# autonomousvision/unimatch

Measured on AMD Instinct MI355X. Metric: image_pairs_per_sec, higher is better.
Workload: dtype f16x2

## Files before the change

include/unimatch_hip.h:

```cpp
#ifndef UNIMATCH_HIP_H
#define UNIMATCH_HIP_H

#include <stddef.h>
#include <stdint.h>

#ifdef __cplusplus
extern "C" {
#endif

#define UM_VERSION 220

#define UM_MODE_EXACT 0
#define UM_MODE_FAST 1

#define UM_ERR_BAD_ARG (-1)
#define UM_ERR_BAD_GEOMETRY (-2)
#define UM_ERR_WORKSPACE (-3)
#define UM_ERR_UNSUPPORTED (-4)
#define UM_ERR_COLLECTIVE (-5)

int um_version(void);
const char* um_last_error_string(void);

#define UM_RANGE_PLANES 1u
// ... 82 lines not shown

int um_linear_bias_fwd(const float* a0, const void* a_planes, const void* w_planes, const float* bias, int m, int n, int k,
                       int wshift, float out_mul, float bias_mul, void* out_planes, float* out_f32, int mode, void* stream);

int um_ffn_fwd(const float* x, const float* y, const void* w1_planes, const void* w2_planes, int m, int hidden,
               int wshift, const float* gamma, const float* beta, float eps, float* out, int mode, void* stream);
size_t um_ffn_split_workspace_bytes(int m, int hidden);
int um_ffn_ws_fwd(const float* x, const float* y, const void* w1_planes, const void* w2_planes, int m, int hidden,
                  int wshift, const float* gamma, const float* beta, float eps, float* out, int mode, void* workspace,
                  size_t workspace_bytes, void* stream);

int um_kv4_fwd(const float* x, const void* wc_planes, int m, int wshift, void* out_planes, int mode, void* stream);
int um_ffn_kv_fwd(const float* x, const float* y, const void* w1_planes, const void* w2_planes, int m, int hidden, int wshift,
                  const float* gamma, const float* beta, float eps, float* out, const void* wc_planes, void* kv_planes, int mode,
                  void* workspace, size_t workspace_bytes, void* stream);

int um_conv2d_fwd(const void* a_planes, const void* w_planes, const float* bias, float* out, float* stats_out, int batch,
                  int hi, int wi, int cin, int cout, int kh, int kw, int stride, int pad_h, int pad_w, int relu, int wshift,
                  int mode, void* stream);
int um_conv2d_ex(const void* a_planes, int a_ld, int a_coff, long a_rows, const void* w_planes, const float* bias, float* out,
                 int out_ld, int out_coff, void* out_planes, int outp_ld, int outp_coff, long outp_rows, float* stats_out,
                 int batch, int hi, int wi, int cin, int cout, int kh, int kw, int stride, int pad_h, int pad_w, int act,
                 int wshift, int mode, void* stream);
int um_conv2d_gru_fwd(int gate, const void* a_planes, int a_ld, int a_coff, long a_rows, const void* w_planes, const float* bias,
                      float* hidden, const float* z, int z_ld, float* z_out, int z_out_ld, void* out_planes, int outp_ld,
                      int outp_coff, long outp_rows, int batch, int hi, int wi, int cin, int channels, int kh, int kw, int pad_h,
                      int pad_w, int wshift, int mode, void* stream);
int um_conv2d_gru_add_fwd(int gate, const void* a_planes, int a_ld, int a_coff, long a_rows, const void* w_planes, const float* bias,
                          const float* addend, int addend_ld, float* hidden, const float* z, int z_ld, float* z_out, int z_out_ld,
                          void* out_planes, int outp_ld, int outp_coff, long outp_rows, int batch, int hi, int wi, int cin,
// ... 229 lines not shown
```

unimatch_amd/_abi.py:

```python
import ctypes
import os

_HERE = os.path.dirname(os.path.abspath(__file__))
LIB_PATH = os.environ.get('UM_LIB') or os.path.join(_HERE, 'libunimatch_hip.so')

MODE_EXACT = 0
MODE_FAST = 1

CENSUS = {'wattn_tile': 0, 'wattn_ksplit': 1, 'ffn_tile': 2, 'ffn_hsplit': 3, 'gsv4': 4, 'gsv3': 5, 'k4_mfma': 6, 'k4_valu': 7,
          'k3_mfma': 8, 'k3_valu': 9, 'conv_patch': 10, 'conv_rows': 11, 'conv_generic': 12, 'wattn_w8': 13, 'conv_patch_norm': 14}

_c_int, _c_size_t, _c_void_p = ctypes.c_int, ctypes.c_size_t, ctypes.c_void_p

SIGNATURES = {
    'um_version': (_c_int, []),
    'um_last_error_string': (ctypes.c_char_p, []),
    'um_range_flags': (_c_int, [ctypes.POINTER(ctypes.c_uint), _c_int]),
    'um_timing_enable': (_c_int, [_c_int]),
    'um_timing_collect': (_c_int, [_c_int, ctypes.POINTER(ctypes.c_double), ctypes.POINTER(_c_int)]),
    'um_window_attn_workspace_bytes': (_c_size_t, [_c_int] * 4),
    'um_window_attn_fwd': (_c_int, [_c_void_p] * 4 + [_c_int] * 9 + [_c_void_p, _c_size_t, _c_void_p]),
    'um_window_attn_planes_fwd': (_c_int, [_c_void_p] * 4 + [_c_int] * 6 + [ctypes.c_long] * 2 + [_c_int] * 6 + [_c_void_p]),
    'um_window_attn_merge_fwd': (_c_int, [_c_void_p] * 7 + [ctypes.c_float, _c_int, _c_void_p] + [_c_int] * 6 + [ctypes.c_long] * 2 +
                                 [_c_int] * 6 + [_c_void_p]),
    'um_window_attn_qproj_merge_fwd': (_c_int, [_c_void_p] * 8 + [ctypes.c_float, _c_int, _c_void_p] + [_c_int] * 5 + [ctypes.c_long] +
                                       [_c_int] * 6 + [_c_void_p, _c_size_t, _c_void_p]),
    'um_window_attn_ksplit_workspace_bytes': (_c_size_t, [_c_int] * 5),
    'um_window_attn_plan': (_c_int, [_c_int] * 5 + [ctypes.POINTER(_c_int)] * 3),
    'um_planes_bytes': (_c_size_t, [ctypes.c_long, _c_int, _c_int]),
    'um_weight_planes': (_c_int, [_c_void_p] * 2 + [_c_int] * 4 + [_c_void_p]),
    'um_linear_fwd': (_c_int, [_c_void_p] * 4 + [_c_int] * 5 + [_c_void_p] * 4 + [ctypes.c_float, _c_int, _c_void_p]),
    'um_linear_bias_fwd': (_c_int, [_c_void_p] * 4 + [_c_int] * 4 + [ctypes.c_float] * 2 + [_c_void_p] * 2 + [_c_int, _c_void_p]),
    'um_ffn_fwd': (_c_int, [_c_void_p] * 4 + [_c_int] * 3 + [_c_void_p] * 2 + [ctypes.c_float, _c_void_p, _c_int, _c_void_p]),
    'um_ffn_ws_fwd': (_c_int, [_c_void_p] * 4 + [_c_int] * 3 + [_c_void_p] * 2 + [ctypes.c_float, _c_void_p, _c_int, _c_void_p, _c_size_t,
                                _c_void_p]),
    'um_ffn_split_workspace_bytes': (_c_size_t, [_c_int] * 2),
    'um_ffn_kv_fwd': (_c_int, [_c_void_p] * 4 + [_c_int] * 3 + [_c_void_p] * 2 + [ctypes.c_float, _c_void_p, _c_void_p, _c_void_p, _c_int, _c_void_p,
                                _c_size_t, _c_void_p]),
    'um_kv4_fwd': (_c_int, [_c_void_p, _c_void_p, _c_int, _c_int, _c_void_p, _c_int, _c_void_p]),
    'um_conv2d_fwd': (_c_int, [_c_void_p] * 5 + [_c_int] * 13 + [_c_void_p]),
    'um_conv2d_addend_fwd': (_c_int, [_c_void_p] * 4 + [_c_int, _c_int, _c_void_p] + [_c_int] * 12 + [_c_void_p]),
    'um_conv2d_ex': (_c_int, [_c_void_p, _c_int, _c_int, ctypes.c_long, _c_void_p, _c_void_p, _c_void_p, _c_int, _c_int, _c_void_p,
                              _c_int, _c_int, ctypes.c_long, _c_void_p] + [_c_int] * 13 + [_c_void_p]),
    'um_nhwc_gate': (_c_int, [_c_int, _c_void_p, _c_int, _c_void_p, _c_void_p, _c_void_p, _c_int, _c_int, ctypes.c_long, ctypes.c_long,
                              _c_int, _c_void_p]),
    'um_local_corr_with_flow_planes': (_c_int, [_c_void_p] * 4 + [_c_int, ctypes.c_long] + [_c_int] * 5 + [_c_void_p]),
    'um_conv2d_gru_fwd': (_c_int, [_c_int, _c_void_p, _c_int, _c_int, ctypes.c_long, _c_void_p, _c_void_p, _c_void_p, _c_void_p, _c_int,
                                   _c_void_p, _c_int, _c_void_p, _c_int, _c_int, ctypes.c_long] + [_c_int] * 11 + [_c_void_p]),
    'um_conv2d_gru_add_fwd': (_c_int, [_c_int, _c_void_p, _c_int, _c_int, ctypes.c_long, _c_void_p, _c_void_p, _c_void_p, _c_int, _c_void_p, _c_void_p,
                                        _c_int, _c_void_p, _c_int, _c_void_p, _c_int, _c_int, ctypes.c_long] + [_c_int] * 11 + [_c_void_p]),
    'um_conv2d_norm_supported': (_c_int, [_c_int] * 10),
    'um_conv2d_norm_fwd': (_c_int, [_c_void_p, _c_void_p, _c_int] + [_c_void_p] * 4 + [_c_int] * 13 + [_c_void_p]),
    'um_conv2d_entry_supported': (_c_int, [_c_int] * 10),
# ... 188 lines not shown
```

unimatch_amd/csrc/ffn.hip:

```cpp
#include <type_traits>
#include <stdlib.h>
#include "common.h"
#include "planes.h"

#ifdef UM_FFN_TRACE
__device__ unsigned long long* g_um_ffn_trace = nullptr;
#define UM_FSTAMP(slot) do { if (tracing && i < 24) trace_buf[(i) * 8 + (slot)] = __builtin_amdgcn_s_memtime(); } while (0)
#else
#define UM_FSTAMP(slot) do { } while (0)
#endif

struct Kv4Args {
    const float* x;
    const unsigned short* w;
    long w_plane_stride;
    unsigned short* out;
    long out_plane_stride;
    int M;
    float out_scale;
    unsigned* range_flag;
};

struct FfnArgs {
    const float* x;
// ... 1 lines not shown
    const unsigned short* w1;
    long w1_plane_stride;
    const unsigned short* w2;
    long w2_plane_stride;
    const float* gamma;
    const float* beta;
    float* out;
    int M, hid;
    float out_scale;
    float eps;
    int split;
    float* hs_part;
    unsigned* hs_flag;
    Kv4Args kv;
    unsigned* range_flag;
};

#ifndef UM_FFN_PRIO
#define UM_FFN_PRIO 0
#endif
#ifndef UM_FFN_ABL
#define UM_FFN_ABL 0
#endif
struct Gelu2 {
    float x[2], r[2];
};
#define UM_GELU_STAGES 4
__device__ __forceinline__ void ffn_gelu_stage(Gelu2& g, int stage) {
#pragma unroll
    for (int i = 0; i < 2; ++i) {
// ... 168 lines not shown
            if (NS == 2) {
                const u32x4 l = {T::lo2(v0[0], v0[1], h[0], neg1), T::lo2(v0[2], v0[3], h[1], neg1),
                                 T::lo2(v1[0], v1[1], h[2], neg1), T::lo2(v1[2], v1[3], h[3], neg1)};
                yf[NS - 1][ks] = __builtin_bit_cast(i16x8, l);
            }
        }
        um_range_note<T>(k.range_flag, xmx, UM_RANGE_KV_TOKENS);
    }
    const int arow = tl ^ (16 * role);
    int aoff[8];
#pragma unroll
    for (int ks = 0; ks < 8; ++ks) aoff[ks] = arow * 512 + (((16 * role + 2 * ks + half) ^ arow) << 4);
    kv4_project<T, NS, false>(lds, lds + Kv4Lds<NS>::RING, k, yf, m0, wave, lane, aoff, neg1);
}

template <typename T, int NS, bool HSPLIT = false, bool KV4 = false>
__global__ __launch_bounds__(512, 2) void ffn_kernel(FfnArgs a) {
    using L = FfnLds<NS>;
    extern __shared__ __attribute__((aligned(16))) unsigned char lds[];

    const int tid = threadIdx.x, lane = tid & 63;
    const float neg1 = um_opaque_neg1();
    const int wave = __builtin_amdgcn_readfirstlane(tid >> 6);
    const int pair = wave & 3, role = wave >> 2;
    const int half = lane >> 5, tl = lane & 31;
    const int nsplit = HSPLIT ? a.split : 1;
    const int tile_id = HSPLIT ? (int)blockIdx.x / nsplit : (int)blockIdx.x;
    const int part = HSPLIT ? (int)blockIdx.x - tile_id * nsplit : 0;
    const int m0 = tile_id * 128;
    const int tok = m0 + 32 * pair + tl;
    const int nslice = (a.hid >> 5) / nsplit;
// ... 489 lines not shown
            for (int g = 0; g < 4; ++g) {
                const int n = 32 * ot + 8 * g;
                const f32x4 gm = *reinterpret_cast<const f32x4*>(a.gamma + n + 4 * half);
                const f32x4 bt = *reinterpret_cast<const f32x4*>(a.beta + n + 4 * half);
                f32x4 yv;
#pragma unroll
                for (int i = 0; i < 4; ++i) yv[i] = (o[ot][4 * g + i] - mean) * rstd * gm[i] + bt[i] + rr[4 * ot + g][i];
                *reinterpret_cast<f32x4*>(stg + tl * 512 + (((8 * ot + 2 * g + half) ^ tl) << 4)) = yv;
                if constexpr (KV4) {
#pragma unroll
                    for (int i = 0; i < 4; ++i) o[ot][4 * g + i] = yv[i];
                }
            }
        __builtin_amdgcn_wave_barrier();
        const int cc = lane & 31;
#pragma unroll
        for (int j = 0; j < 16; ++j) {
            const int r = 2 * j + half;
            const f32x4 v = *reinterpret_cast<const f32x4*>(stg + r * 512 + ((cc ^ r) << 4));
            const int trow = m0 + 32 * pair + r;
            if (trow < a.M) *reinterpret_cast<f32x4*>(a.out + (long)trow * 128 + 4 * cc) = v;
        }
    }
#ifdef UM_FFN_TRACE
    if (tracing) trace_buf[24 * 8 + 2] = __builtin_amdgcn_s_memtime();
#endif
    if constexpr (KV4) {
        i16x8 yf[NS][8];
        unsigned char* xch = lds + 65536 + pair * 16384 + lane * 16;
        if (role == 0) {
#pragma unroll
            for (int ot = 0; ot < 4; ++ot)
#pragma unroll
                for (int kk = 0; kk < 2; ++kk) {
                    unsigned wh[4], wl[4];
#pragma unroll
                    for (int j = 0; j < 4; ++j) {
// ... 28 lines not shown
        }
        kv4_project<T, NS, true>(lds, lds + 65536, a.kv, yf, m0, wave, lane, aoff, neg1);
#ifdef UM_FFN_TRACE
        if (tracing) trace_buf[24 * 8 + 3] = __builtin_amdgcn_s_memtime();
#endif
    }
}

extern void um_set_error(const char* fmt, ...);
#ifdef UM_FFN_TRACE
extern "C" int um_debug_set_ffn_trace(void* ptr) {
    return (int)hipMemcpyToSymbol(HIP_SYMBOL(g_um_ffn_trace), &ptr, sizeof(ptr));
}
#endif

template <typename T, int NS, bool HSPLIT, bool KV4 = false>
static hipError_t launch_ffn_impl(const FfnArgs& a, hipStream_t stream) {
    constexpr int LDS = FfnLds<NS>::TOTAL > 131072 ? FfnLds<NS>::TOTAL : (KV4 ? 131072 : FfnLds<NS>::TOTAL);
    static bool configured = false;
    if (!configured) {
        hipError_t e = hipFuncSetAttribute(reinterpret_cast<const void*>(&ffn_kernel<T, NS, HSPLIT, KV4>),
                                           hipFuncAttributeMaxDynamicSharedMemorySize, LDS);
        if (e != hipSuccess) return e;
        configured = true;
    }
    ScopedKernelTimer timer(UM_K_FFN, stream);
    um_census_hit(HSPLIT ? UM_V_FFN_HSPLIT : UM_V_FFN_TILE);
    hipLaunchKernelGGL((ffn_kernel<T, NS, HSPLIT, KV4>), dim3(((a.M + 127) / 128) * a.split), dim3(512), LDS, stream, a);
    return hipGetLastError();
}

template <typename T, int NS>
static hipError_t launch_ffn(const FfnArgs& a, hipStream_t stream) {
    if (a.kv.w) return launch_ffn_impl<T, NS, false, true>(a, stream);
    return a.split > 1 ? launch_ffn_impl<T, NS, true>(a, stream) : launch_ffn_impl<T, NS, false>(a, stream);
}

static int ffn_num_cus() { return um_num_cus(); }

static int ffn_hidden_split(int m, int hidden) {
    static const bool off = um_debug_env("UM_FFN_NO_HSPLIT") != nullptr;
    if (off) return 1;
    const int tiles = (m + 127) / 128, nslice = hidden / 32, cus = ffn_num_cus();
    int split = 1;
    while (split < 4 && tiles * (2 * split) <= cus && nslice % (2 * split) == 0 && nslice / (2 * split) >= 4) split *= 2;
    return split;
}

static size_t ffn_hs_bytes(int m, int split) {
// ... 8 lines not shown
}

extern "C" int um_ffn_ws_fwd(const float* x, const float* y, const void* w1_planes, const void* w2_planes, int m, int hidden,
                             int wshift, const float* gamma, const float* beta, float eps, float* out, int mode, void* workspace,
                             size_t workspace_bytes, void* stream_);

extern "C" int um_ffn_fwd(const float* x, const float* y, const void* w1_planes, const void* w2_planes, int m, int hidden,
                          int wshift, const float* gamma, const float* beta, float eps, float* out, int mode,
                          void* stream_) {
    return um_ffn_ws_fwd(x, y, w1_planes, w2_planes, m, hidden, wshift, gamma, beta, eps, out, mode, nullptr, 0, stream_);
}

extern "C" int um_kv4_fwd(const float* x, const void* wc_planes, int m, int wshift, void* out_planes, int mode, void* stream_);
static int ffn_impl(const float* x, const float* y, const void* w1_planes, const void* w2_planes, int m, int hidden,
                    int wshift, const float* gamma, const float* beta, float eps, float* out, int mode, void* workspace,
                    size_t workspace_bytes, const void* wc_planes, void* kv_planes, void* stream_);

extern "C" int um_ffn_ws_fwd(const float* x, const float* y, const void* w1_planes, const void* w2_planes, int m, int hidden,
                             int wshift, const float* gamma, const float* beta, float eps, float* out, int mode, void* workspace,
                             size_t workspace_bytes, void* stream_) {
    return ffn_impl(x, y, w1_planes, w2_planes, m, hidden, wshift, gamma, beta, eps, out, mode, workspace, workspace_bytes, nullptr,
                    nullptr, stream_);
}

extern "C" int um_ffn_kv_fwd(const float* x, const float* y, const void* w1_planes, const void* w2_planes, int m, int hidden,
                             int wshift, const float* gamma, const float* beta, float eps, float* out, const void* wc_planes,
                             void* kv_planes, int mode, void* workspace, size_t workspace_bytes, void* stream_) {
    if (!wc_planes || !kv_planes) {
        um_set_error("um_ffn_kv_fwd: null k | v weight planes or output planes");
        return -1;
    }
    return ffn_impl(x, y, w1_planes, w2_planes, m, hidden, wshift, gamma, beta, eps, out, mode, workspace, workspace_bytes, wc_planes,
                    kv_planes, stream_);
}

static int ffn_impl(const float* x, const float* y, const void* w1_planes, const void* w2_planes, int m, int hidden,
                    int wshift, const float* gamma, const float* beta, float eps, float* out, int mode, void* workspace,
                    size_t workspace_bytes, const void* wc_planes, void* kv_planes, void* stream_) {
    if (!x || !y || !w1_planes || !w2_planes || !gamma || !beta || !out || m <= 0 || hidden < 64 || hidden % 32 != 0 ||
        (mode != 0 && mode != 1) || wshift < 0 || wshift > 14) {
        um_set_error("um_ffn_fwd: bad argument (m=%d hidden=%d wshift=%d mode=%d; hidden must be a multiple of 32, >= 64)",
                     m, hidden, wshift, mode);
        return -1;
    }
    if ((long)hidden * 256 * 2 >= (1L << 32)) {
        um_set_error("um_ffn_fwd: weight planes beyond 4 GiB are not addressable by this kernel");
        return -4;
    }
    FfnArgs a;
    a.x = x;
    a.y = y;
    a.w1 = (const unsigned short*)w1_planes;
    a.w1_plane_stride = (long)hidden * 256;
    a.w2 = (const unsigned short*)w2_planes;
    a.w2_plane_stride = (long)128 * hidden;
    a.gamma = gamma;
    a.beta = beta;
    a.out = out;
    a.M = m;
    a.hid = hidden;
    a.out_scale = ldexpf(1.f, -wshift);
    a.eps = eps;
    a.split = 1;
    a.hs_part = nullptr;
    a.hs_flag = nullptr;
    a.kv = Kv4Args{};
    a.range_flag = a.kv.range_flag = (mode == 0) ? um_range_flag_dev() : nullptr;
    if (workspace) {
        const int split = ffn_hidden_split(m, hidden);
        if (split > 1 && workspace_bytes >= ffn_hs_bytes(m, split)) {
            const size_t slots = (size_t)((m + 127) / 128);
            a.split = split;
            a.hs_flag = (unsigned*)workspace;
            a.hs_part = (float*)((unsigned char*)workspace + ((slots * sizeof(unsigned) + 255) & ~(size_t)255));
        }
    }
    static const bool no_fuse = um_debug_env("UM_FFN_NO_KV4") != nullptr;
    const bool fuse = wc_planes && a.split == 1 && !no_fuse;
    if (fuse) {
        a.kv.x = nullptr;
        a.kv.w = (const unsigned short*)wc_planes;
        a.kv.w_plane_stride = 256L * 256;
        a.kv.out = (unsigned short*)kv_planes;
        a.kv.out_plane_stride = 4L * m * 128;
        a.kv.M = m;
        a.kv.out_scale = a.out_scale;
    }
    const hipError_t e = mode == 0 ? launch_ffn<Fp16, 2>(a, (hipStream_t)stream_) : launch_ffn<Bf16, 1>(a, (hipStream_t)stream_);
    if (e != hipSuccess) {
        um_set_error("um_ffn_fwd: launch failed: %s", hipGetErrorString(e));
        return (int)e;
    }
    if (wc_planes && !fuse) return um_kv4_fwd(out, wc_planes, m, wshift, kv_planes, mode, stream_);
    return 0;
}

extern "C" int um_kv4_fwd(const float* x, const void* wc_planes, int m, int wshift, void* out_planes, int mode, void* stream_) {
    if (!x || !wc_planes || !out_planes || m <= 0 || (mode != 0 && mode != 1) || wshift < 0 || wshift > 14) {
        um_set_error("um_kv4_fwd: bad argument (m=%d wshift=%d mode=%d)", m, wshift, mode);
        return -1;
    }
    Kv4Args k;
    k.x = x;
    k.w = (const unsigned short*)wc_planes;
    k.w_plane_stride = 256L * 256;
    k.out = (unsigned short*)out_planes;
    k.out_plane_stride = 4L * m * 128;
    k.M = m;
// ... 32 lines not shown
```

unimatch_amd/model.py:

```python
import math
import weakref

import torch
import torch.nn as nn
import torch.nn.functional as F

from .encoder import CNNEncoder
from .refine import BasicUpdateBlock, convex_upsample
from .refine_nhwc import NhwcUpdateBlock
from .dist import shard_batch, shard_bounds
from .streams import PartRunner, forward_parts
from .confidence import depth_match_confidence, match_confidence

_IMAGENET_MEAN = (0.485, 0.456, 0.406)
_IMAGENET_STD = (0.229, 0.224, 0.225)


def attention_windows(attn_type, is_self, splits, h, w, with_shift):
    if attn_type == 'swin':
        kind = 'win2d'
    elif attn_type == 'self_swin2d_cross_1d':
        kind = 'win2d' if is_self else 'row'
    elif attn_type == 'self_swin2d_cross_swin1d':
        kind = 'win2d' if is_self else 'winrow'
# ... 40 lines not shown
class TransformerLayer(nn.Module):

    def __init__(self, d_model, no_ffn, ffn_dim_expansion):
        super().__init__()
        self.q_proj = nn.Linear(d_model, d_model, bias=False)
        self.k_proj = nn.Linear(d_model, d_model, bias=False)
        self.v_proj = nn.Linear(d_model, d_model, bias=False)
        self.merge = nn.Linear(d_model, d_model, bias=False)
        self.norm1 = nn.LayerNorm(d_model)
        self.no_ffn = no_ffn
        if not no_ffn:
            self.mlp = nn.Sequential(nn.Linear(2 * d_model, 2 * d_model * ffn_dim_expansion, bias=False), nn.GELU(),
                                     nn.Linear(2 * d_model * ffn_dim_expansion, d_model, bias=False))
            self.norm2 = nn.LayerNorm(d_model)

    def forward(self, ops, source, target, h, w, geom, kv_rotate=0, kv=None, next_kv_weights=None):
        if getattr(ops, 'fused_tail', False):
            return self._forward_fused(ops, source, target, h, w, geom, kv_rotate, kv, next_kv_weights)
        assert kv_rotate == 0 and kv is None and next_kv_weights is None
        q, k, v = self.q_proj(source), self.k_proj(target), self.v_proj(target)
        msg = ops.window_attention(q, k, v, h, w, *geom)
        msg = self.norm1(self.merge(msg))
        if not self.no_ffn:
            msg = self.norm2(self.mlp(torch.cat([source, msg], dim=-1)))
        return source + msg

    def _forward_fused(self, ops, source, target, h, w, geom, kv_rotate=0, kv=None, next_kv_weights=None):
        s, l, c = source.shape
        m = s * l
        src = source.reshape(m, c)
        if getattr(ops, 'fused_qproj', False) and getattr(ops, 'fused_merge', False):
            if kv is None:
                kvp, _, n2 = ops.linear_planes(target.reshape(m, c), (self.k_proj.weight, self.v_proj.weight))
                koff, voff = 0, c
                kop, vop = (kvp, m, n2, koff), (kvp, m, n2, voff)
            else:
                kop, vop = kv
                assert kop[1] == m
            res = src if self.no_ffn else None
            msg = ops.window_attention_qproj_merge(src, self.q_proj.weight, kop, vop, s, h, w, *geom,
                                                   kv_rotate, self.merge.weight, self.norm1, res)
            if self.no_ffn:
                return msg
            msg = msg.reshape(m, c)
            if next_kv_weights is not None:
                out, nkv = ops.ffn_ln_kv(src, msg, self.mlp[0].weight, self.mlp[2].weight, self.norm2, next_kv_weights)
                return out.reshape(s, l, c), nkv
            if getattr(ops, 'fused_ffn', False):
                return ops.ffn_ln(src, msg, self.mlp[0].weight, self.mlp[2].weight, self.norm2).reshape(s, l, c)
            hid, _, nh = ops.linear_planes(src, (self.mlp[0].weight,), a1=msg, gelu=True)
            return ops.linear_ln(hid, (self.mlp[2].weight,), self.norm2, residual=src, a_planes_k=nh).reshape(s, l, c)
        assert kv is None and next_kv_weights is None, 'precomputed k | v planes need the fused q-projection / merge path'
        if target is source:
            qkv, _, n3 = ops.linear_planes(src, (self.q_proj.weight, self.k_proj.weight, self.v_proj.weight))
            q, k, v = (qkv, m, n3, 0), (qkv, m, n3, c), (qkv, m, n3, 2 * c)
        else:
            qp, _, _ = ops.linear_planes(src, (self.q_proj.weight,))
            kv, _, n2 = ops.linear_planes(target.reshape(m, c), (self.k_proj.weight, self.v_proj.weight))
            q, k, v = (qp, m, c, 0), (kv, m, n2, 0), (kv, m, n2, c)
        if getattr(ops, 'fused_merge', False):
            res = src if self.no_ffn else None
            msg = ops.window_attention_merge(q, k, v, s, h, w, *geom, kv_rotate, self.merge.weight, self.norm1, res)
            if self.no_ffn:
                return msg
            msg = msg.reshape(m, c)
        else:
            att = ops.window_attention_planes(q, k, v, s, h, w, *geom, kv_rotate=kv_rotate).reshape(m, c)
# ... 20 lines not shown
        if nhead != 1:
            raise NotImplementedError('multi-head attention is not implemented (neither does the reference, '
                                      'transformer.py:63-66)')
        self.d_model = d_model
        self.layers = nn.ModuleList([TransformerBlock(d_model, ffn_dim_expansion) for _ in range(num_layers)])
        for p in self.parameters():
            if p.dim() > 1:
                nn.init.xavier_uniform_(p)

    def forward(self, ops, tok0, tok1, h, w, attn_type, attn_num_splits, stream=None):
        if stream is None:
            stream = torch.cat([tok0, tok1], 0)
        b = stream.shape[0] // 2
        rotate = getattr(ops, 'fused_tail', False)
        prev = stream if rotate else torch.cat([stream[b:], stream[:b]], 0)
        block_kv = rotate and getattr(ops, 'fused_qproj', False) and getattr(ops, 'fused_merge', False) and getattr(ops, 'block_kv', True)
        s2, l, c = stream.shape
        fused_kv = block_kv and getattr(ops, 'fused_kv', False) and getattr(ops, 'fused_ffn', False)
        kv4 = None
        kvw = lambda b_: (b_.self_attn.k_proj.weight, b_.self_attn.v_proj.weight, b_.cross_attn_ffn.k_proj.weight,
                          b_.cross_attn_ffn.v_proj.weight)
        for i, blk in enumerate(self.layers):
            shift = ('swin' in attn_type) and attn_num_splits > 1 and i % 2 == 1
            g_self = attention_windows(attn_type, True, attn_num_splits, h, w, shift)
            g_cross = attention_windows(attn_type, False, attn_num_splits, h, w, shift)
            kv_s = kv_c = None
            if block_kv:
                if kv4 is None:
                    kv4 = ops.kv4_planes(stream.reshape(s2 * l, c), kvw(blk))
                kv_s, kv_c = ops.kv4_slices(kv4, s2 * l)
                kv4 = None
            stream = blk.self_attn(ops, stream, stream, h, w, g_self, kv=kv_s)
            if rotate:
                nxt = kvw(self.layers[i + 1]) if fused_kv and i + 1 < len(self.layers) else None
                stream = blk.cross_attn_ffn(ops, stream, prev, h, w, g_cross, kv_rotate=b, kv=kv_c, next_kv_weights=nxt)
                if nxt is not None:
                    stream, kv4 = stream
                prev = stream
            else:
                stream = blk.cross_attn_ffn(ops, stream, prev, h, w, g_cross)
                prev = torch.cat([stream[b:], stream[:b]], 0)
        return stream[:b].contiguous(), stream[b:].contiguous()


class SelfAttnPropagation(nn.Module):

    def __init__(self, in_channels):
        super().__init__()
        self.q_proj = nn.Linear(in_channels, in_channels)
        self.k_proj = nn.Linear(in_channels, in_channels)
        for p in self.parameters():
            if p.dim() > 1:
# ... 811 lines not shown
```

unimatch_amd/ops.py:

```python
import contextlib
import ctypes
import threading
import weakref
from collections import namedtuple

import torch

from . import _abi

PRECISIONS = {'exact': _abi.MODE_EXACT, 'fast': _abi.MODE_FAST}


class KernelTimer:

    def __init__(self):
        self.records = []

    def summary(self):
        torch.cuda.synchronize()
        out = {}
        for name, s, e, meta in self.records:
            d = out.setdefault(name, {'calls': 0, 'ms': 0.0, 'meta': meta})
            d['calls'] += 1
            d['ms'] += s.elapsed_time(e)
# ... 16 lines not shown
        raise ValueError(f'{name}: shape {tuple(t.shape)} does not match N={n}, L={tokens}')


def _check_map(name, t, n, h, w):
    if not (t.is_cuda and t.dtype == torch.float32 and t.dim() == 4 and t.is_contiguous()
            and t.shape[0] == n and t.shape[2] == h and t.shape[3] == w):
        raise ValueError(f'{name}: expected a contiguous CUDA float32 [{n}, V, {h}, {w}] tensor, got '
                         f'{tuple(t.shape)} {t.dtype}')


def pack_kv4_weights(weights):
    w4 = torch.cat([w.detach().float() for w in weights], 0)
    perm = torch.arange(32, device=w4.device) ^ 16
    cross = w4[256:].view(8, 32, 128)[:, perm].reshape(256, 128)
    return torch.cat([w4[:256], cross], 1).contiguous()


WorkspaceKey = namedtuple('WorkspaceKey', 'kind geometry device owner')


class _Scope(threading.local):
    token = None
    lane = 0


class WorkspaceRegistry:

    GEOMETRIES = 8

    def __init__(self, stream=None, capturing=None):
# ... 41 lines not shown
        return buf

    def release_cached_planes(self):
        for k in [k for k in self._entries if isinstance(k.kind, tuple)]:
            del self._entries[k]


class HipOps(WorkspaceRegistry):

    fused_tail = True
    fused_ffn = True
    fused_merge = True
    fused_qproj = True
    block_kv = True
    refine_hoist = True
    fused_kv = True
    fused_conv = True
    norm_on_load = True
    fused_entry = True
    fused_glue = True
    CONV_MODE = 0
    WSHIFT = 10

    def __init__(self, precision='exact'):
        if precision not in PRECISIONS:
            raise ValueError(f'precision must be one of {sorted(PRECISIONS)}')
        self.lib = _abi.load()
        if not torch.cuda.is_available():
            raise _abi.HipExtensionError('no GPU visible: the UniMatch hot path only runs on the HIP extension')
        self.precision = precision
        self.mode = PRECISIONS[precision]
# ... 53 lines not shown
        self.cache_generation += 1
        return value

    def weight_planes(self, weights):
        key, hit = self._cache_get('lin', weights)
        if hit is not None:
            return hit
        w = (weights[0] if len(weights) == 1 else torch.cat(list(weights), 0)).detach().float().contiguous()
        n, k = w.shape
        self._check_weight_range(w, self.WSHIFT if self.mode == 0 else 0, 'Linear weight')
        planes = torch.empty(self.lib.um_planes_bytes(n, k, self.mode), dtype=torch.uint8, device=w.device)
        _abi.check(self.lib.um_weight_planes(_ptr(w), _ptr(planes), n, k, self.WSHIFT, self.mode, _stream()),
                   'um_weight_planes')
        return self._cache_put(key, weights, (planes, n, k))

    @staticmethod
    def _check_weight_range(w, shift, what):
        limit = 65504.0 / float(1 << shift)
        amax = float(w.abs().max()) if w.numel() else 0.0
        if not amax < limit:
            raise ValueError(f'{what}: max |w| = {amax:.4g} does not fit the fp16 operand planes (|w| < {limit:.4g} at the '
                             f'2^{shift} pre-scale; see include/unimatch_hip.h, "Operand range")')

    def _check_rows(self, name, t, k):
        if not (t.is_cuda and t.dtype == torch.float32 and t.dim() == 2 and t.is_contiguous() and t.shape[1] == k):
            raise ValueError(f'{name}: expected a contiguous CUDA float32 [M, {k}] tensor, got {tuple(t.shape)} {t.dtype}')

    def linear_planes(self, a, weights, a1=None, gelu=False, a_planes_k=None):
        wp, n, k = self.weight_planes(weights)
        if a_planes_k is not None:
            m = a.numel() // (2 * self.nplanes * a_planes_k)
            args = (None, None, _ptr(a))
        else:
            m = a.shape[0]
            self._check_rows('a', a, k // 2 if a1 is not None else k)
            if a1 is not None:
                self._check_rows('a1', a1, k // 2)
            args = (_ptr(a), _ptr(a1) if a1 is not None else None, None)
        out = torch.empty(self.lib.um_planes_bytes(m, n, self.mode), dtype=torch.uint8, device=a.device)
        meta = {'flops': 2.0 * m * n * k}
        code = self._launch('linear', lambda: self.lib.um_linear_fwd(
            args[0], args[1], args[2], _ptr(wp), m, n, k, self.WSHIFT, 2 if gelu else 0, _ptr(out),
            None, None, None, 0.0, self.mode, _stream()), meta)
# ... 7 lines not shown
            args = (None, None, _ptr(a))
        else:
            m = a.shape[0]
            self._check_rows('a', a, k)
            args = (_ptr(a), None, None)
        if residual is not None:
            self._check_rows('residual', residual, n)
        out = torch.empty((m, n), dtype=torch.float32, device=a.device)
        code = self._launch('linear', lambda: self.lib.um_linear_fwd(
            args[0], args[1], args[2], _ptr(wp), m, n, k, self.WSHIFT, 1, _ptr(out),
            _ptr(norm.weight), _ptr(norm.bias), _ptr(residual) if residual is not None else None,
            float(norm.eps), self.mode, _stream()), {'flops': 2.0 * m * n * k})
        _abi.check(code, 'um_linear_fwd')
        return out

    def ffn_ln(self, x, y, w1, w2, norm):
        w1p, hid, k1 = self.weight_planes((w1,))
        w2p, n2, k2 = self.weight_planes((w2,))
        if (k1, n2, k2) != (256, 128, hid):
            raise ValueError(f'ffn_ln: expected W1 [hidden, 256] and W2 [128, hidden], got {tuple(w1.shape)} {tuple(w2.shape)}')
        self._check_rows('x', x, 128)
        self._check_rows('y', y, 128)
        m = x.shape[0]
        if y.shape[0] != m:
            raise ValueError('ffn_ln: x and y must have the same number of rows')
        out = torch.empty((m, 128), dtype=torch.float32, device=x.device)
        ws = self._split_workspace('ffn_hsplit', (m, hid), x.device)
        code = self._launch('ffn', lambda: self.lib.um_ffn_ws_fwd(
            _ptr(x), _ptr(y), _ptr(w1p), _ptr(w2p), m, hid, self.WSHIFT, _ptr(norm.weight), _ptr(norm.bias),
            float(norm.eps), _ptr(out), self.mode, _ptr(ws) if ws is not None else None, ws.numel() if ws is not None else 0,
            _stream()), {'flops': 2.0 * m * hid * (256 + 128)})
        _abi.check(code, 'um_ffn_ws_fwd')
        return out

    def ffn_ln_kv(self, x, y, w1, w2, norm, kv_weights):
        w1p, hid, k1 = self.weight_planes((w1,))
        w2p, n2, k2 = self.weight_planes((w2,))
        if (k1, n2, k2) != (256, 128, hid):
            raise ValueError(f'ffn_ln_kv: expected W1 [hidden, 256] and W2 [128, hidden], got {tuple(w1.shape)} {tuple(w2.shape)}')
        self._check_rows('x', x, 128)
        self._check_rows('y', y, 128)
        m = x.shape[0]
# ... 36 lines not shown
        out = torch.empty((streams, h * w, 128), dtype=torch.float32, device=qt.device)
        meta = {'flops': 4.0 * streams * h * w * win_h * win_w * 128}
        code = self._launch('window_attn', lambda: self.lib.um_window_attn_merge_fwd(
            _ptr(qt) + 2 * qoff, _ptr(kt) + 2 * koff, _ptr(vt) + 2 * voff, _ptr(wp), _ptr(norm.weight), _ptr(norm.bias),
            _ptr(residual) if residual is not None else None, float(norm.eps), self.WSHIFT, _ptr(out), streams, h, w, 128,
            qcols, kcols, qrows * qcols, krows * kcols, win_h, win_w, shift_h, shift_w, kv_rotate, self.mode, _stream()), meta)
        _abi.check(code, 'um_window_attn_merge_fwd')
        return out

    def _split_workspace(self, kind, geometry, device):
        size = self.lib.um_window_attn_ksplit_workspace_bytes if kind == 'attn_ksplit' else self.lib.um_ffn_split_workspace_bytes
        nbytes = size(*geometry)
        return self._workspace(kind, geometry, nbytes, device, self.GEOMETRIES) if nbytes else None

    def window_attention_qproj_merge(self, x, q_weight, k, v, streams, h, w, win_h, win_w, shift_h, shift_w, kv_rotate,
                                     merge_weight, norm, residual=None):
        (kt, krows, kcols, koff), (vt, vrows, vcols, voff) = k[:4], v[:4]
        kps = k[4] if len(k) > 4 else krows * kcols
        if (v[4] if len(v) > 4 else vrows * vcols) != kps:
            raise ValueError('k and v must share their plane stride')
        self._check_rows('x', x, 128)
        if (krows, kcols) != (vrows, vcols) or x.shape[0] != streams * h * w or krows != x.shape[0]:
            raise ValueError('inconsistent plane shapes')
        wqp, nq, kq = self.weight_planes((q_weight,))
        wp, n, kk = self.weight_planes((merge_weight,))
        if (n, kk, nq, kq) != (128, 128, 128, 128):
            raise ValueError('window_attention_qproj_merge: the query and merge weights must be [128, 128]')
        if residual is not None:
            self._check_rows('residual', residual, 128)
        out = torch.empty((streams, h * w, 128), dtype=torch.float32, device=x.device)
        meta = {'flops': 4.0 * streams * h * w * win_h * win_w * 128}
        ks = self._split_workspace('attn_ksplit', (streams, h, w, win_h, win_w), x.device)
        code = self._launch('window_attn', lambda: self.lib.um_window_attn_qproj_merge_fwd(
            _ptr(x), _ptr(wqp), _ptr(kt) + 2 * koff, _ptr(vt) + 2 * voff, _ptr(wp), _ptr(norm.weight), _ptr(norm.bias),
            _ptr(residual) if residual is not None else None, float(norm.eps), self.WSHIFT, _ptr(out), streams, h, w, 128,
            kcols, kps, win_h, win_w, shift_h, shift_w, kv_rotate, self.mode,
            _ptr(ks) if ks is not None else None, ks.numel() if ks is not None else 0, _stream()), meta)
        _abi.check(code, 'um_window_attn_qproj_merge_fwd')
# ... 916 lines not shown
```

Baseline: 983.6.

## Fold K/V projections into query and merge weights, emit FFN output planes

Folds the key projection into the query weight (Wk^T·Wq) and the value projection into the merge weight (Wm·Wv), so attention reads the raw stream planes and no per-layer K/V projection GEMM is needed. The FFN kernel gains a PLANES variant that writes fp16/bf16 split planes of its output in the epilogue, and these become the next layer's K/V input. The folded layer path is turned on by default and the fused_kv path is turned off. The folded weights are computed in double precision and cached, but reassociating the products changes rounding and may raise the dynamic range that the plane quantisation must cover.

Result: faster. 1034, median of 6 (+5.2%).

```diff
diff --git a/include/unimatch_hip.h b/include/unimatch_hip.h
--- a/include/unimatch_hip.h
+++ b/include/unimatch_hip.h
@@ -120,6 +120,9 @@
 int um_ffn_kv_fwd(const float* x, const float* y, const void* w1_planes, const void* w2_planes, int m, int hidden, int wshift,
                   const float* gamma, const float* beta, float eps, float* out, const void* wc_planes, void* kv_planes, int mode,
                   void* workspace, size_t workspace_bytes, void* stream);
+int um_ffn_planes_fwd(const float* x, const float* y, const void* w1_planes, const void* w2_planes, int m, int hidden, int wshift,
+                      const float* gamma, const float* beta, float eps, float* out, void* out_planes, int mode, void* workspace,
+                      size_t workspace_bytes, void* stream);
 
 int um_conv2d_fwd(const void* a_planes, const void* w_planes, const float* bias, float* out, float* stats_out, int batch,
                   int hi, int wi, int cin, int cout, int kh, int kw, int stride, int pad_h, int pad_w, int relu, int wshift,
diff --git a/unimatch_amd/_abi.py b/unimatch_amd/_abi.py
--- a/unimatch_amd/_abi.py
+++ b/unimatch_amd/_abi.py
@@ -37,6 +37,8 @@
     'um_ffn_split_workspace_bytes': (_c_size_t, [_c_int] * 2),
     'um_ffn_kv_fwd': (_c_int, [_c_void_p] * 4 + [_c_int] * 3 + [_c_void_p] * 2 + [ctypes.c_float, _c_void_p, _c_void_p, _c_void_p, _c_int, _c_void_p,
                                 _c_size_t, _c_void_p]),
+    'um_ffn_planes_fwd': (_c_int, [_c_void_p] * 4 + [_c_int] * 3 + [_c_void_p] * 2 + [ctypes.c_float, _c_void_p, _c_void_p, _c_int, _c_void_p, _c_size_t,
+                                    _c_void_p]),
     'um_kv4_fwd': (_c_int, [_c_void_p, _c_void_p, _c_int, _c_int, _c_void_p, _c_int, _c_void_p]),
     'um_conv2d_fwd': (_c_int, [_c_void_p] * 5 + [_c_int] * 13 + [_c_void_p]),
     'um_conv2d_addend_fwd': (_c_int, [_c_void_p] * 4 + [_c_int, _c_int, _c_void_p] + [_c_int] * 12 + [_c_void_p]),
diff --git a/unimatch_amd/csrc/ffn.hip b/unimatch_amd/csrc/ffn.hip
--- a/unimatch_amd/csrc/ffn.hip
+++ b/unimatch_amd/csrc/ffn.hip
@@ -39,6 +39,8 @@
     unsigned* hs_flag;
     Kv4Args kv;
     unsigned* range_flag;
+    unsigned short* planes;
+    long planes_stride;
 };
 
 #ifndef UM_FFN_PRIO
@@ -237,7 +239,7 @@
     kv4_project<T, NS, false>(lds, lds + Kv4Lds<NS>::RING, k, yf, m0, wave, lane, aoff, neg1);
 }
 
-template <typename T, int NS, bool HSPLIT = false, bool KV4 = false>
+template <typename T, int NS, bool HSPLIT = false, bool KV4 = false, bool PLANES = false>
 __global__ __launch_bounds__(512, 2) void ffn_kernel(FfnArgs a) {
     using L = FfnLds<NS>;
     extern __shared__ __attribute__((aligned(16))) unsigned char lds[];
@@ -757,13 +759,25 @@
             }
         __builtin_amdgcn_wave_barrier();
         const int cc = lane & 31;
+        float pmx = 0.f;
 #pragma unroll
         for (int j = 0; j < 16; ++j) {
             const int r = 2 * j + half;
             const f32x4 v = *reinterpret_cast<const f32x4*>(stg + r * 512 + ((cc ^ r) << 4));
             const int trow = m0 + 32 * pair + r;
-            if (trow < a.M) *reinterpret_cast<f32x4*>(a.out + (long)trow * 128 + 4 * cc) = v;
-        }
+            if (trow < a.M) {
+                *reinterpret_cast<f32x4*>(a.out + (long)trow * 128 + 4 * cc) = v;
+                if constexpr (PLANES) {
+                    pmx = fmaxf(fmaxf(pmx, fmaxf(__builtin_fabsf(v[0]), __builtin_fabsf(v[1]))), fmaxf(__builtin_fabsf(v[2]), __builtin_fabsf(v[3])));
+                    unsigned short* pp = a.planes + (long)trow * 128 + 4 * cc;
+                    const unsigned h0 = T::pack2(v[0], v[1]), h1 = T::pack2(v[2], v[3]);
+                    *reinterpret_cast<u32x2*>(pp) = u32x2{h0, h1};
+                    if (NS == 2)
+                        *reinterpret_cast<u32x2*>(pp + a.planes_stride) = u32x2{T::lo2(v[0], v[1], h0, neg1), T::lo2(v[2], v[3], h1, neg1)};
+                }
+            }
+        }
+        if constexpr (PLANES) um_range_note<T>(a.range_flag, pmx, UM_RANGE_KV_TOKENS);
     }
 #ifdef UM_FFN_TRACE
     if (tracing) trace_buf[24 * 8 + 2] = __builtin_amdgcn_s_memtime();
@@ -822,25 +836,26 @@
 }
 #endif
 
-template <typename T, int NS, bool HSPLIT, bool KV4 = false>
+template <typename T, int NS, bool HSPLIT, bool KV4 = false, bool PLANES = false>
 static hipError_t launch_ffn_impl(const FfnArgs& a, hipStream_t stream) {
     constexpr int LDS = FfnLds<NS>::TOTAL > 131072 ? FfnLds<NS>::TOTAL : (KV4 ? 131072 : FfnLds<NS>::TOTAL);
     static bool configured = false;
     if (!configured) {
-        hipError_t e = hipFuncSetAttribute(reinterpret_cast<const void*>(&ffn_kernel<T, NS, HSPLIT, KV4>),
+        hipError_t e = hipFuncSetAttribute(reinterpret_cast<const void*>(&ffn_kernel<T, NS, HSPLIT, KV4, PLANES>),
                                            hipFuncAttributeMaxDynamicSharedMemorySize, LDS);
         if (e != hipSuccess) return e;
         configured = true;
     }
     ScopedKernelTimer timer(UM_K_FFN, stream);
     um_census_hit(HSPLIT ? UM_V_FFN_HSPLIT : UM_V_FFN_TILE);
-    hipLaunchKernelGGL((ffn_kernel<T, NS, HSPLIT, KV4>), dim3(((a.M + 127) / 128) * a.split), dim3(512), LDS, stream, a);
+    hipLaunchKernelGGL((ffn_kernel<T, NS, HSPLIT, KV4, PLANES>), dim3(((a.M + 127) / 128) * a.split), dim3(512), LDS, stream, a);
     return hipGetLastError();
 }
 
 template <typename T, int NS>
 static hipError_t launch_ffn(const FfnArgs& a, hipStream_t stream) {
     if (a.kv.w) return launch_ffn_impl<T, NS, false, true>(a, stream);
+    if (a.planes) return launch_ffn_impl<T, NS, false, false, true>(a, stream);
     return a.split > 1 ? launch_ffn_impl<T, NS, true>(a, stream) : launch_ffn_impl<T, NS, false>(a, stream);
 }
 
@@ -879,13 +894,13 @@
 extern "C" int um_kv4_fwd(const float* x, const void* wc_planes, int m, int wshift, void* out_planes, int mode, void* stream_);
 static int ffn_impl(const float* x, const float* y, const void* w1_planes, const void* w2_planes, int m, int hidden,
                     int wshift, const float* gamma, const float* beta, float eps, float* out, int mode, void* workspace,
-                    size_t workspace_bytes, const void* wc_planes, void* kv_planes, void* stream_);
+                    size_t workspace_bytes, const void* wc_planes, void* kv_planes, void* out_planes, void* stream_);
 
 extern "C" int um_ffn_ws_fwd(const float* x, const float* y, const void* w1_planes, const void* w2_planes, int m, int hidden,
                              int wshift, const float* gamma, const float* beta, float eps, float* out, int mode, void* workspace,
                              size_t workspace_bytes, void* stream_) {
     return ffn_impl(x, y, w1_planes, w2_planes, m, hidden, wshift, gamma, beta, eps, out, mode, workspace, workspace_bytes, nullptr,
-                    nullptr, stream_);
+                    nullptr, nullptr, stream_);
 }
 
 extern "C" int um_ffn_kv_fwd(const float* x, const float* y, const void* w1_planes, const void* w2_planes, int m, int hidden,
@@ -896,12 +911,23 @@
         return -1;
     }
     return ffn_impl(x, y, w1_planes, w2_planes, m, hidden, wshift, gamma, beta, eps, out, mode, workspace, workspace_bytes, wc_planes,
-                    kv_planes, stream_);
+                    kv_planes, nullptr, stream_);
+}
+
+extern "C" int um_ffn_planes_fwd(const float* x, const float* y, const void* w1_planes, const void* w2_planes, int m, int hidden,
+                                 int wshift, const float* gamma, const float* beta, float eps, float* out, void* out_planes, int mode,
+                                 void* workspace, size_t workspace_bytes, void* stream_) {
+    if (!out_planes) {
+        um_set_error("um_ffn_planes_fwd: null output planes");
+        return -1;
+    }
+    return ffn_impl(x, y, w1_planes, w2_planes, m, hidden, wshift, gamma, beta, eps, out, mode, workspace, workspace_bytes, nullptr,
+                    nullptr, out_planes, stream_);
 }
 
 static int ffn_impl(const float* x, const float* y, const void* w1_planes, const void* w2_planes, int m, int hidden,
                     int wshift, const float* gamma, const float* beta, float eps, float* out, int mode, void* workspace,
-                    size_t workspace_bytes, const void* wc_planes, void* kv_planes, void* stream_) {
+                    size_t workspace_bytes, const void* wc_planes, void* kv_planes, void* out_planes, void* stream_) {
     if (!x || !y || !w1_planes || !w2_planes || !gamma || !beta || !out || m <= 0 || hidden < 64 || hidden % 32 != 0 ||
         (mode != 0 && mode != 1) || wshift < 0 || wshift > 14) {
         um_set_error("um_ffn_fwd: bad argument (m=%d hidden=%d wshift=%d mode=%d; hidden must be a multiple of 32, >= 64)",
@@ -930,6 +956,8 @@
     a.hs_part = nullptr;
     a.hs_flag = nullptr;
     a.kv = Kv4Args{};
+    a.planes = nullptr;
+    a.planes_stride = (long)m * 128;
     a.range_flag = a.kv.range_flag = (mode == 0) ? um_range_flag_dev() : nullptr;
     if (workspace) {
         const int split = ffn_hidden_split(m, hidden);
@@ -951,12 +979,20 @@
         a.kv.M = m;
         a.kv.out_scale = a.out_scale;
     }
+    if (out_planes && a.split == 1) a.planes = (unsigned short*)out_planes;
     const hipError_t e = mode == 0 ? launch_ffn<Fp16, 2>(a, (hipStream_t)stream_) : launch_ffn<Bf16, 1>(a, (hipStream_t)stream_);
     if (e != hipSuccess) {
         um_set_error("um_ffn_fwd: launch failed: %s", hipGetErrorString(e));
         return (int)e;
     }
     if (wc_planes && !fuse) return um_kv4_fwd(out, wc_planes, m, wshift, kv_planes, mode, stream_);
+    if (out_planes && !a.planes) {
+        const hipError_t es = launch_split_planes(out, (unsigned short*)out_planes, m, 1.f, mode, (hipStream_t)stream_);
+        if (es != hipSuccess) {
+            um_set_error("um_ffn_planes_fwd: format pass failed: %s", hipGetErrorString(es));
+            return (int)es;
+        }
+    }
     return 0;
 }
 
diff --git a/unimatch_amd/model.py b/unimatch_amd/model.py
--- a/unimatch_amd/model.py
+++ b/unimatch_amd/model.py
@@ -78,10 +78,10 @@
                                      nn.Linear(2 * d_model * ffn_dim_expansion, d_model, bias=False))
             self.norm2 = nn.LayerNorm(d_model)
 
-    def forward(self, ops, source, target, h, w, geom, kv_rotate=0, kv=None, next_kv_weights=None):
+    def forward(self, ops, source, target, h, w, geom, kv_rotate=0, kv=None, next_kv_weights=None, fold=False, next_planes=False):
         if getattr(ops, 'fused_tail', False):
-            return self._forward_fused(ops, source, target, h, w, geom, kv_rotate, kv, next_kv_weights)
-        assert kv_rotate == 0 and kv is None and next_kv_weights is None
+            return self._forward_fused(ops, source, target, h, w, geom, kv_rotate, kv, next_kv_weights, fold, next_planes)
+        assert kv_rotate == 0 and kv is None and next_kv_weights is None and not fold and not next_planes
         q, k, v = self.q_proj(source), self.k_proj(target), self.v_proj(target)
         msg = ops.window_attention(q, k, v, h, w, *geom)
         msg = self.norm1(self.merge(msg))
@@ -89,11 +89,12 @@
             msg = self.norm2(self.mlp(torch.cat([source, msg], dim=-1)))
         return source + msg
 
-    def _forward_fused(self, ops, source, target, h, w, geom, kv_rotate=0, kv=None, next_kv_weights=None):
+    def _forward_fused(self, ops, source, target, h, w, geom, kv_rotate=0, kv=None, next_kv_weights=None, fold=False, next_planes=False):
         s, l, c = source.shape
         m = s * l
         src = source.reshape(m, c)
         if getattr(ops, 'fused_qproj', False) and getattr(ops, 'fused_merge', False):
+            assert not fold or (kv is not None and next_kv_weights is None), 'the folded layer reads the planes of the stream itself'
             if kv is None:
                 kvp, _, n2 = ops.linear_planes(target.reshape(m, c), (self.k_proj.weight, self.v_proj.weight))
                 koff, voff = 0, c
@@ -102,11 +103,18 @@
                 kop, vop = kv
                 assert kop[1] == m
             res = src if self.no_ffn else None
-            msg = ops.window_attention_qproj_merge(src, self.q_proj.weight, kop, vop, s, h, w, *geom,
-                                                   kv_rotate, self.merge.weight, self.norm1, res)
+            if fold:
+                msg = ops.window_attention_qproj_merge(src, self.q_proj.weight, kop, vop, s, h, w, *geom, kv_rotate, self.merge.weight,
+                                                       self.norm1, res, fold=(self.k_proj.weight, self.v_proj.weight))
+            else:
+                msg = ops.window_attention_qproj_merge(src, self.q_proj.weight, kop, vop, s, h, w, *geom,
+                                                       kv_rotate, self.merge.weight, self.norm1, res)
             if self.no_ffn:
                 return msg
             msg = msg.reshape(m, c)
+            if next_planes:
+                out, npl = ops.ffn_ln(src, msg, self.mlp[0].weight, self.mlp[2].weight, self.norm2, planes=True)
+                return out.reshape(s, l, c), npl
             if next_kv_weights is not None:
                 out, nkv = ops.ffn_ln_kv(src, msg, self.mlp[0].weight, self.mlp[2].weight, self.norm2, next_kv_weights)
                 return out.reshape(s, l, c), nkv
@@ -114,7 +122,8 @@
                 return ops.ffn_ln(src, msg, self.mlp[0].weight, self.mlp[2].weight, self.norm2).reshape(s, l, c)
             hid, _, nh = ops.linear_planes(src, (self.mlp[0].weight,), a1=msg, gelu=True)
             return ops.linear_ln(hid, (self.mlp[2].weight,), self.norm2, residual=src, a_planes_k=nh).reshape(s, l, c)
-        assert kv is None and next_kv_weights is None, 'precomputed k | v planes need the fused q-projection / merge path'
+        assert kv is None and next_kv_weights is None and not fold and not next_planes, \
+            'precomputed k | v planes need the fused q-projection / merge path'
         if target is source:
             qkv, _, n3 = ops.linear_planes(src, (self.q_proj.weight, self.k_proj.weight, self.v_proj.weight))
             q, k, v = (qkv, m, n3, 0), (qkv, m, n3, c), (qkv, m, n3, 2 * c)
@@ -165,8 +174,12 @@
         b = stream.shape[0] // 2
         rotate = getattr(ops, 'fused_tail', False)
         prev = stream if rotate else torch.cat([stream[b:], stream[:b]], 0)
-        block_kv = rotate and getattr(ops, 'fused_qproj', False) and getattr(ops, 'fused_merge', False) and getattr(ops, 'block_kv', True)
+        fused_attn = rotate and getattr(ops, 'fused_qproj', False) and getattr(ops, 'fused_merge', False)
         s2, l, c = stream.shape
+        fold = fused_attn and getattr(ops, 'fold_kv', False)
+        fold_ffn = fold and getattr(ops, 'fused_ffn', False)
+        planes = None
+        block_kv = fused_attn and not fold and getattr(ops, 'block_kv', True)
         fused_kv = block_kv and getattr(ops, 'fused_kv', False) and getattr(ops, 'fused_ffn', False)
         kv4 = None
         kvw = lambda b_: (b_.self_attn.k_proj.weight, b_.self_attn.v_proj.weight, b_.cross_attn_ffn.k_proj.weight,
@@ -176,17 +189,26 @@
             g_self = attention_windows(attn_type, True, attn_num_splits, h, w, shift)
             g_cross = attention_windows(attn_type, False, attn_num_splits, h, w, shift)
             kv_s = kv_c = None
+            if fold:
+                if planes is None:
+                    planes, _, _ = ops.linear_planes(stream.reshape(s2 * l, c), ())
+                kv_s = kv_c = ((planes, s2 * l, c, 0),) * 2
+                planes = None
             if block_kv:
                 if kv4 is None:
                     kv4 = ops.kv4_planes(stream.reshape(s2 * l, c), kvw(blk))
                 kv_s, kv_c = ops.kv4_slices(kv4, s2 * l)
                 kv4 = None
-            stream = blk.self_attn(ops, stream, stream, h, w, g_self, kv=kv_s)
+            stream = blk.self_attn(ops, stream, stream, h, w, g_self, kv=kv_s, fold=fold)
             if rotate:
                 nxt = kvw(self.layers[i + 1]) if fused_kv and i + 1 < len(self.layers) else None
-                stream = blk.cross_attn_ffn(ops, stream, prev, h, w, g_cross, kv_rotate=b, kv=kv_c, next_kv_weights=nxt)
+                nxp = fold_ffn and i + 1 < len(self.layers)
+                stream = blk.cross_attn_ffn(ops, stream, prev, h, w, g_cross, kv_rotate=b, kv=kv_c, next_kv_weights=nxt, fold=fold,
+                                            next_planes=nxp)
                 if nxt is not None:
                     stream, kv4 = stream
+                elif nxp:
+                    stream, planes = stream
                 prev = stream
             else:
                 stream = blk.cross_attn_ffn(ops, stream, prev, h, w, g_cross)
diff --git a/unimatch_amd/ops.py b/unimatch_amd/ops.py
--- a/unimatch_amd/ops.py
+++ b/unimatch_amd/ops.py
@@ -54,6 +54,15 @@
     perm = torch.arange(32, device=w4.device) ^ 16
     cross = w4[256:].view(8, 32, 128)[:, perm].reshape(256, 128)
     return torch.cat([w4[:256], cross], 1).contiguous()
+
+
+def fold_weights(kind, a, b):
+    a, b = a.detach().double(), b.detach().double()
+    if kind == 'q':
+        a = a.t()
+    elif kind != 'm':
+        raise ValueError(f"fold_weights: kind must be 'q' or 'm', got {kind!r}")
+    return (a.unsqueeze(2) * b.unsqueeze(0)).sum(1).float().contiguous()
 
 
 WorkspaceKey = namedtuple('WorkspaceKey', 'kind geometry device owner')
@@ -125,7 +134,8 @@
     fused_qproj = True
     block_kv = True
     refine_hoist = True
-    fused_kv = True
+    fused_kv = False
+    fold_kv = True
     fused_conv = True
     norm_on_load = True
     fused_entry = True
@@ -209,6 +219,14 @@
                    'um_weight_planes')
         return self._cache_put(key, weights, (planes, n, k))
 
+    def _folded_weight(self, kind, a, b):
+        key, hit = self._cache_get('fold_' + kind, (a, b))
+        if hit is not None:
+            return hit
+        if tuple(a.shape) != (128, 128) or tuple(b.shape) != (128, 128):
+            raise ValueError('folded attention weights: expected two [128, 128] weights')
+        return self._cache_put(key, (a, b), fold_weights(kind, a, b))
+
     @staticmethod
     def _check_weight_range(w, shift, what):
         limit = 65504.0 / float(1 << shift)
@@ -222,6 +240,15 @@
             raise ValueError(f'{name}: expected a contiguous CUDA float32 [M, {k}] tensor, got {tuple(t.shape)} {t.dtype}')
 
     def linear_planes(self, a, weights, a1=None, gelu=False, a_planes_k=None):
+        if len(weights) == 0:
+            if a1 is not None or gelu or a_planes_k is not None or not (a.dim() == 2 and a.shape[0] > 0):
+                raise ValueError('linear_planes: the identity takes one fp32 [M, K] tensor and no epilogue')
+            m, k = a.shape
+            self._check_rows('a', a, k)
+            out = torch.empty(self.lib.um_planes_bytes(m, k, self.mode), dtype=torch.uint8, device=a.device)
+            _abi.check(self._launch('split_planes', lambda: self.lib.um_weight_planes(_ptr(a), _ptr(out), m, k, 0, self.mode, _stream())),
+                       'um_weight_planes')
+            return out, m, k
         wp, n, k = self.weight_planes(weights)
         if a_planes_k is not None:
             m = a.numel() // (2 * self.nplanes * a_planes_k)
@@ -259,7 +286,7 @@
         _abi.check(code, 'um_linear_fwd')
         return out
 
-    def ffn_ln(self, x, y, w1, w2, norm):
+    def ffn_ln(self, x, y, w1, w2, norm, planes=False):
         w1p, hid, k1 = self.weight_planes((w1,))
         w2p, n2, k2 = self.weight_planes((w2,))
         if (k1, n2, k2) != (256, 128, hid):
@@ -271,6 +298,14 @@
             raise ValueError('ffn_ln: x and y must have the same number of rows')
         out = torch.empty((m, 128), dtype=torch.float32, device=x.device)
         ws = self._split_workspace('ffn_hsplit', (m, hid), x.device)
+        if planes:
+            pl = torch.empty(self.lib.um_planes_bytes(m, 128, self.mode), dtype=torch.uint8, device=x.device)
+            code = self._launch('ffn', lambda: self.lib.um_ffn_planes_fwd(
+                _ptr(x), _ptr(y), _ptr(w1p), _ptr(w2p), m, hid, self.WSHIFT, _ptr(norm.weight), _ptr(norm.bias),
+                float(norm.eps), _ptr(out), _ptr(pl), self.mode, _ptr(ws) if ws is not None else None,
+                ws.numel() if ws is not None else 0, _stream()), {'flops': 2.0 * m * hid * (256 + 128)})
+            _abi.check(code, 'um_ffn_planes_fwd')
+            return out, pl
         code = self._launch('ffn', lambda: self.lib.um_ffn_ws_fwd(
             _ptr(x), _ptr(y), _ptr(w1p), _ptr(w2p), m, hid, self.WSHIFT, _ptr(norm.weight), _ptr(norm.bias),
             float(norm.eps), _ptr(out), self.mode, _ptr(ws) if ws is not None else None, ws.numel() if ws is not None else 0,
@@ -337,7 +372,7 @@
         return self._workspace(kind, geometry, nbytes, device, self.GEOMETRIES) if nbytes else None
 
     def window_attention_qproj_merge(self, x, q_weight, k, v, streams, h, w, win_h, win_w, shift_h, shift_w, kv_rotate,
-                                     merge_weight, norm, residual=None):
+                                     merge_weight, norm, residual=None, fold=None):
         (kt, krows, kcols, koff), (vt, vrows, vcols, voff) = k[:4], v[:4]
         kps = k[4] if len(k) > 4 else krows * kcols
         if (v[4] if len(v) > 4 else vrows * vcols) != kps:
@@ -345,6 +380,8 @@
         self._check_rows('x', x, 128)
         if (krows, kcols) != (vrows, vcols) or x.shape[0] != streams * h * w or krows != x.shape[0]:
             raise ValueError('inconsistent plane shapes')
+        if fold is not None:
+            q_weight, merge_weight = self._folded_weight('q', fold[0], q_weight), self._folded_weight('m', merge_weight, fold[1])
         wqp, nq, kq = self.weight_planes((q_weight,))
         wp, n, kk = self.weight_planes((merge_weight,))
         if (n, kk, nq, kq) != (128, 128, 128, 128):
```
